# Audio-WestlakeU/FN-SSL

Measured on AMD Instinct MI355X. Metric: TF-frames/sec DP-IPD forward, 4-mic 257-bin x 300-frame, higher is better.
Workload: dtype f32; 1 GPU; BASELINE configs[1]: FN-SSL (online) DP-IPD forward, waveform->STFT->features->3x(full-band BiLSTM + narrow-band LSTM)->head; 32 utterances/GPU x 4 mics ('MM' = 6 pairs) x 257 bins x 300 frames, fp32; frame = one STFT frame of one utterance; stream_chunk_frames=0, utterances_per_gpu=32, global_batch=32, mics=4, pairs_per_utterance=6, frames=300, bins=257, parallelism=dp1 (utterance shards, no collective), chunk_pairs=0

## Files before the change

fn-ssl_amd/csrc/lstm_f32c.h:

```cpp
#pragma once

#include "lstm_static.h"

namespace fnssl_lstm {

constexpr int kF32cWaves = 16;

struct F32ClusterParams {
  unsigned* tags;
  unsigned* status;
  int clusters_per_dir;
  int groups_per_cluster;
  unsigned spin_limit;
  int stall_member;
  int rotate;
  int prio_mode;
};

template <int HH, int NV0, int NS0, int MODE, bool ABLRT = false, int DRIFT = 2, int NW_ = kF32cWaves, int GS = 1>
__global__ void __launch_bounds__(NW_ * 64) lstm_f32c_kernel(const LstmParams p, const F32ClusterParams cp) {
  constexpr int H = HH, NS = H / 16, NW = NW_;
  constexpr int NWS = NW / GS;
  static_assert((GS == 1 || GS == 4) && NW % GS == 0 && (NWS & (NWS - 1)) == 0, "gate split: whole slots, a power of two of them");
  constexpr bool SUM = (MODE & kSum) != 0, SAVE = (MODE & kSave) != 0;
  constexpr bool CAT = (MODE & kHas2) != 0;
  constexpr int QPS = 1 + NV0 + NS0 + NS;
  constexpr int XD = NW_ > 12 ? 4 : 8;
  constexpr bool STRH = H == 256 && GS == 1 && NW_ > 8;
  static_assert((CAT ? NS0 == 1 : !(NV0 && NS0)) && (NV0 == 0 || NV0 % XD == 0) && (H == 128 || H == 256),
                "blocks of src0, or its remainder alone, or blocks of src0 + the remainder quad of src2");
  static_assert(H == 128 || NW_ <= 8 || STRH, "H = 256 with the row of h_{t-1} held: at most two waves per SIMD (register budget)");
  static_assert(!STRH || (NV0 >= XD && (NV0 + NS) % XD == 0), "streamed row: the ring depth divides the block count");
  static_assert(GS == 1 || (!SAVE && !ABLRT), "gate split: inference kernels only");
  extern __shared__ __attribute__((aligned(16))) char smem[];
  const int ABL = ABLRT ? p.ablate : 0;

  const int b = blockIdx.x;
  const int m = (b >> 3) % NS;
  const int cl = ((b >> 3) / NS) * 8 + (b & 7);
  if (cl >= cp.clusters_per_dir * p.ndir) return;
  const int dir = cl / cp.clusters_per_dir;
  const int ck = cl - dir * cp.clusters_per_dir;
  const int g0 = ck * cp.groups_per_cluster;
  const int g1 = g0 + cp.groups_per_cluster < p.ntasks ? g0 + cp.groups_per_cluster : p.ntasks;
  if (__hip_atomic_load(cp.status, __ATOMIC_RELAXED, __HIP_MEMORY_SCOPE_AGENT) != 0) return;
  if (cl == 0 && m == cp.stall_member) return;

  const int lane = threadIdx.x & 63;
  const int n = lane & 15, g = lane >> 4;
  const int w = __builtin_amdgcn_readfirstlane((int)(threadIdx.x >> 6));
  const int ws = GS == 1 ? w : (w >> 2);
  const int gate = GS == 1 ? 0 : (w & 3);
  const bool rev = dir == 1;
  const unsigned vlane = lane * 16;

  {
    const v4f* src = reinterpret_cast<const v4f*>(reinterpret_cast<const char*>(p.wpack[dir]) + (size_t)(m * QPS) * 4096);
    v4f* dst = reinterpret_cast<v4f*>(smem);
    for (int i = threadIdx.x; i < QPS * 4 * 64; i += NW * 64) dst[i] = src[i];
  }
  char* const xch = smem + QPS * 4096;
  unsigned* const xcnt = reinterpret_cast<unsigned*>(xch + NWS * 2 * 4 * 1024);
  if (GS > 1 && threadIdx.x < NWS) xcnt[threadIdx.x] = 0;
  __syncthreads();
  const char* const lds_rd = smem + lane * 16;
  auto rec = [&](int q, int j) { return *reinterpret_cast<const v4f*>(lds_rd + (q * 4 + j) * 1024); };
  auto rec1 = [&](int q, int j) { return *reinterpret_cast<const float*>(lds_rd + (q * 4 + j) * 1024 + 4 * gate); };

  const unsigned st0 = (unsigned)(p.src0.st * 4), sto = (unsigned)(p.out_st * 4), stk = SUM ? (unsigned)(p.skip.st * 4) : 0u;
  const unsigned st2 = CAT ? (unsigned)(p.src2.st * 4) : 0u;
  const unsigned cy = (unsigned)p.carry;
  unsigned* const tag_cl = cp.tags + (size_t)cl * cp.groups_per_cluster * NS;
  const v4f zero4 = v4f{0.f, 0.f, 0.f, 0.f};

  unsigned pub_val = 0;
  unsigned* pub_tag = nullptr;
  auto pub_flush = [&]() {
    if (pub_tag) {
      asm volatile("s_waitcnt vmcnt(0)" ::: "memory");
      if (lane == 0) __hip_atomic_store(pub_tag, pub_val, __ATOMIC_RELAXED, __HIP_MEMORY_SCOPE_AGENT);
      pub_tag = nullptr;
    }
  };

  struct Grp {
    unsigned vo0, voo, vok, voo2, vo2 = 0;
    bool valid;
    int task, step;
  };
  auto locate = [&](int task, int qo0, int qi0, Grp& gr, rsrc_t& rx0, rsrc_t& ro, rsrc_t& rsk, rsrc_t& ro2, rsrc_t& rx2) {
    const int q0 = task * 16;
    gr.valid = q0 + n < p.nseq;
    const int d = q0 + n < p.nseq ? n : p.nseq - 1 - q0;
    const bool crossed = qi0 + d >= p.q_inner;
    auto one = [&](const float* base, long long so, long long si, int extra, unsigned& voff) {
      const long long delta = (long long)d * si + (crossed ? so - (long long)p.q_inner * si : 0ll);
      voff = (unsigned)(delta * 4) + (unsigned)(extra * 4);
      return make_rsrc(base + ((long long)qo0 * so + (long long)qi0 * si));
    };
    rx0 = one(p.src0.p, p.src0.so, p.src0.si, (NS0 && !CAT) ? g : 4 * g, gr.vo0);
    if constexpr (CAT) rx2 = one(p.src2.p, p.src2.so, p.src2.si, g, gr.vo2);
    ro = one(p.out, p.out_so, p.out_si, dir * H + 4 * g, gr.voo);
    gr.vok = gr.voo2 = 0;
    rsk = SUM ? one(p.skip.p, p.skip.so, p.skip.si, dir * H + 4 * g, gr.vok) : rx0;
    ro2 = SUM ? one(p.out_sum, p.out_so, p.out_si, dir * H + 4 * g, gr.voo2) : ro;
  };
  auto tt_of = [&](int step) { return (unsigned)(rev ? p.nsteps - 1 - step : step); };
  auto rc_of = [&](int task) {
    return make_rsrc(cell_record<NS>(p.cscratch, p.ntasks, dir, task));
  };

  if (g0 + ws >= g1) return;
  unsigned long long clk0 = 0, rt0 = 0;
  if (ABLRT && (ABL & 512)) {
    clk0 = __builtin_amdgcn_s_memtime();
    rt0 = __builtin_amdgcn_s_memrealtime();
  }
  bool dead = false;
  auto bounded_wait = [&](auto ready, auto reload, int sleep, unsigned code) {
    for (unsigned spins = 0; !ready(); ++spins) {
      if (GS > 1) __builtin_amdgcn_s_sleep(1); else if (sleep == 8) __builtin_amdgcn_s_sleep(8); else __builtin_amdgcn_s_sleep(16);
      reload();
      const bool out = spins > cp.spin_limit;
      if (out || (spins & 63) == 63) {
        if (out) {
          if (lane == 0) __hip_atomic_store(cp.status, code | (unsigned)(cl & 0xffff), __ATOMIC_RELAXED, __HIP_MEMORY_SCOPE_AGENT);
          return false;
        }
        if (__hip_atomic_load(cp.status, __ATOMIC_RELAXED, __HIP_MEMORY_SCOPE_AGENT) != 0) return false;
      }
    }
    return true;
  };
  const int NGR = g1 - g0;
  const bool rot = cp.rotate && NGR >= 2 * NWS;
  const int FULL = rot ? (NGR / NWS) * NWS : NGR, LEFT = NGR - FULL;
  const bool single = GS == 1 && g0 + ws + NWS >= g1;
  Grp cur, nxt;
  rsrc_t rx0, ro, rsk, ro2, rx2, nrx0, nro, nrsk, nro2, nrx2;
  v4f xr[XD];
  float xs0 = 0.f;
  v4f cprev = zero4, skipv = zero4;
  unsigned tagv = 0, tagd = 0;
  auto request = [&](const Grp& gr, rsrc_t qx0, rsrc_t qsk, bool with_c, bool with_x = true) {
    const unsigned tt = tt_of(gr.step);
    if (!(ABL & 8)) {
      if constexpr (NV0 > 0) if (with_x) static_for<XD>([&](auto v) { xr[v.value] = bld4(qx0, gr.vo0, tt * st0 + 64 * v.value); });
      if constexpr (NS0 > 0 && !CAT) xs0 = bld1(qx0, gr.vo0, tt * st0);
    }
    if (SUM && !(ABL & 64)) skipv = bld4(qsk, gr.vok, tt * stk + 64 * m);
    if (gr.step > 0 || cy) {
      if (gr.step > 0 && !(ABL & 256))
        tagv = __hip_atomic_load(tag_cl + (size_t)(gr.task - g0) * NS + (lane & (NS - 1)), __ATOMIC_RELAXED, __HIP_MEMORY_SCOPE_AGENT);
      if (GS == 1 && with_c && !(ABL & 64)) cprev = bld4_l2(rc_of(gr.task), vlane, m * 1024);
    }
    if (DRIFT > 0 && !(ABL & 256) && gr.task - DRIFT * NWS >= g0)
      tagd = __hip_atomic_load(tag_cl + (size_t)(gr.task - DRIFT * NWS - g0) * NS + (lane & (NS - 1)), __ATOMIC_RELAXED, __HIP_MEMORY_SCOPE_AGENT);
  };
  cur.task = g0 + ws;
  cur.step = 0;
  unsigned iter = 0;
  const int qo_first = (cur.task * 16) / p.q_inner, qi_first = cur.task * 16 - qo_first * p.q_inner;
  int qo0 = qo_first, qi0 = qi_first;
  locate(cur.task, qo0, qi0, cur, rx0, ro, rsk, ro2, rx2);
  request(cur, rx0, rsk, true);
  if constexpr (CAT) xs0 = bld1(rx2, cur.vo2, tt_of(0) * st2);

  for (;;) {
    const int step = cur.step, task = cur.task;
    const unsigned tt = tt_of(step);
    const unsigned o0 = tt * st0, oo = (tt + cy) * sto;
    const unsigned op = (rev ? tt + 1 : tt - 1 + cy) * sto;
    const rsrc_t rc = rc_of(task);
    unsigned* const tag_g = tag_cl + (size_t)(task - g0) * NS;
    if (single && (step > 0 || cy) && !(ABL & 64)) cprev = bld4_l2(rc, vlane, m * 1024);
    const bool late_c = GS > 1 || task >= g0 + FULL;
    v4f cprev_cur = (step > 0 || cy) ? cprev : zero4;
    const v4f skip_cur = skipv;

    v4f hold[STRH ? 1 : NS];
    auto fetch_h = [&]() {
      if (DRIFT > 0 && !(ABL & 4) && !dead && task - DRIFT * NWS >= g0) {
        unsigned* const tag_d = tag_cl + (size_t)(task - DRIFT * NWS - g0) * NS;
        dead = !bounded_wait([&]() { return __builtin_amdgcn_ballot_w64(tagd < (unsigned)step + 1) == 0; },
                             [&]() { tagd = __hip_atomic_load(tag_d + (lane & (NS - 1)), __ATOMIC_RELAXED, __HIP_MEMORY_SCOPE_AGENT); }, 8, 0x40000u);
      }
      if ((step > 0 || cy) && !(ABL & 16)) {
        if (step > 0 && !(ABL & 4) && !dead)
          dead = !bounded_wait([&]() { return __builtin_amdgcn_ballot_w64(tagv < (unsigned)step) == 0; },
                               [&]() { tagv = __hip_atomic_load(tag_g + (lane & (NS - 1)), __ATOMIC_RELAXED, __HIP_MEMORY_SCOPE_AGENT); }, 16, 0x30000u);
        if (late_c && !(ABL & 64)) cprev_cur = bld4_l2(rc, vlane, m * 1024);
        if constexpr (!STRH) {
#pragma unroll
          for (int s = 0; s < NS; ++s) hold[s] = bld4_l2(ro, cur.voo, op + 64 * s);
        }
      } else if constexpr (!STRH) {
#pragma unroll
        for (int s = 0; s < NS; ++s) hold[s] = (ABL & 16) ? cprev : zero4;
      }
    };
    const bool hrow = step > 0 || cy;
    auto hblock = [&](int j) { return hrow ? bld4_l2(ro, cur.voo, op + 64 * j) : zero4; };

    if (cp.prio_mode == 2) __builtin_amdgcn_s_setprio(2);
    v4f acc[4];
    v4f ra[4];
    v4f acc1 = zero4;
    float rb[4] = {0.f, 0.f, 0.f, 0.f};
    if constexpr (GS == 1) {
      acc[0] = rec(0, 0);
      acc[1] = rec(0, 1);
      acc[2] = rec(0, 2);
      acc[3] = rec(0, 3);
      static_for<4>([&](auto j) { ra[j.value] = rec(1, j.value); });
    } else {
      acc1 = rec(0, gate);
      static_for<4>([&](auto j) { rb[j.value] = rec1(1, j.value); });
    }
    auto quad = [&](auto qc, float b0, float b1, float b2, float b3) {
      constexpr int Q = decltype(qc)::value;
      if constexpr (GS > 1) {
        acc1 = __builtin_amdgcn_mfma_f32_16x16x4f32(rb[0], b0, acc1, 0, 0, 0);
        if constexpr (Q + 1 < QPS) rb[0] = rec1(Q + 1, 0);
        acc1 = __builtin_amdgcn_mfma_f32_16x16x4f32(rb[1], b1, acc1, 0, 0, 0);
        if constexpr (Q + 1 < QPS) rb[1] = rec1(Q + 1, 1);
        acc1 = __builtin_amdgcn_mfma_f32_16x16x4f32(rb[2], b2, acc1, 0, 0, 0);
        if constexpr (Q + 1 < QPS) rb[2] = rec1(Q + 1, 2);
        acc1 = __builtin_amdgcn_mfma_f32_16x16x4f32(rb[3], b3, acc1, 0, 0, 0);
        if constexpr (Q + 1 < QPS) rb[3] = rec1(Q + 1, 3);
        return;
      }
      MFMA4(acc, ra[0], b0);
      __builtin_amdgcn_sched_barrier(0);
      if constexpr (Q + 1 < QPS) if (!(ABL & 128)) ra[0] = rec(Q + 1, 0);
      __builtin_amdgcn_sched_barrier(0);
      MFMA4(acc, ra[1], b1);
      __builtin_amdgcn_sched_barrier(0);
      if constexpr (Q + 1 < QPS) if (!(ABL & 128)) ra[1] = rec(Q + 1, 1);
      __builtin_amdgcn_sched_barrier(0);
      MFMA4(acc, ra[2], b2);
      __builtin_amdgcn_sched_barrier(0);
      if constexpr (Q + 1 < QPS) if (!(ABL & 128)) ra[2] = rec(Q + 1, 2);
      __builtin_amdgcn_sched_barrier(0);
      MFMA4(acc, ra[3], b3);
      __builtin_amdgcn_sched_barrier(0);
      if constexpr (Q + 1 < QPS) if (!(ABL & 128)) ra[3] = rec(Q + 1, 3);
      __builtin_amdgcn_sched_barrier(0);
    };
    auto quad1 = [&](auto qc, float b0) {
      constexpr int Q = decltype(qc)::value;
      if constexpr (GS > 1) {
        acc1 = __builtin_amdgcn_mfma_f32_16x16x4f32(rb[0], b0, acc1, 0, 0, 0);
        if constexpr (Q + 1 < QPS) static_for<4>([&](auto j) { rb[j.value] = rec1(Q + 1, j.value); });
        return;
      }
      MFMA4(acc, ra[0], b0);
      if constexpr (Q + 1 < QPS) static_for<4>([&](auto j) { ra[j.value] = rec(Q + 1, j.value); });
    };
    if constexpr (NV0 > 0) {
      static_for<NV0>([&](auto v) {
        constexpr int V = decltype(v)::value;
        if constexpr (STRH) {
          if constexpr (V == NV0 / 2) pub_flush();
          if constexpr (V == NV0 - XD) fetch_h();
        } else if constexpr (V == NV0 / 2) {
          pub_flush();
          fetch_h();
        }
        const v4f xb = xr[V % XD];
        quad(ic<1 + V>{}, xb.x, xb.y, xb.z, xb.w);
        if constexpr (V + XD < NV0) {
          if (!(ABL & 8)) xr[V % XD] = bld4(rx0, cur.vo0, o0 + 64 * (V + XD));
        } else if constexpr (STRH) {
          xr[V % XD] = hblock(V + XD - NV0);
        }
      });
      if constexpr (NS0 > 0) quad1(ic<1 + NV0>{}, xs0);
    } else {
      pub_flush();
      fetch_h();
      quad1(ic<1>{}, xs0);
    }
    bool seq_next = false;
    if (task < g0 + FULL && task + NWS < g0 + FULL) {
      nxt.task = task + NWS;
      nxt.step = step;
      seq_next = true;
    } else {
      const int j = (ws - step) & (NWS - 1);
      if (task < g0 + FULL && j < LEFT) {
        nxt.task = g0 + FULL + j;
        nxt.step = step;
      } else {
        nxt.task = g0 + ws;
        nxt.step = step + 1;
      }
    }
    const bool more = nxt.step < p.nsteps;
    if (more) {
      if (ABL & 1) {
        nxt.vo0 = cur.vo0; nxt.voo = cur.voo; nxt.vok = cur.vok; nxt.voo2 = cur.voo2; nxt.valid = cur.valid;
        nrx0 = rx0; nro = ro; nrsk = rsk; nro2 = ro2;
        if constexpr (CAT) {
          nxt.vo2 = cur.vo2;
          nrx2 = rx2;
        }
      } else {
        if (seq_next) {
          qi0 += 16 * NWS;
          while (qi0 >= p.q_inner) {
            qi0 -= p.q_inner;
            ++qo0;
          }
        } else if (nxt.step == step) {
          qo0 = (nxt.task * 16) / p.q_inner;
          qi0 = nxt.task * 16 - qo0 * p.q_inner;
        } else {
          qo0 = qo_first;
          qi0 = qi_first;
        }
        locate(nxt.task, qo0, qi0, nxt, nrx0, nro, nrsk, nro2, nrx2);
      }
      request(nxt, nrx0, nrsk, !single && nxt.task < g0 + FULL, !STRH);
      if constexpr (CAT) xs0 = bld1(nrx2, nxt.vo2, tt_of(nxt.step) * st2);
    }
    static_for<NS>([&](auto sp) {
      constexpr int SP = decltype(sp)::value;
      if constexpr (STRH) {
        constexpr int B = NV0 + SP, B2 = B + XD;
        const v4f hb = xr[B % XD];
        quad(ic<1 + NV0 + NS0 + SP>{}, hb.x, hb.y, hb.z, hb.w);
        if constexpr (B2 < NV0 + NS) {
          xr[B % XD] = hblock(B2 - NV0);
        } else {
          if (more) xr[B % XD] = bld4(nrx0, nxt.vo0, tt_of(nxt.step) * st0 + 64 * (B2 - NV0 - NS));
        }
      } else {
        quad(ic<1 + NV0 + NS0 + SP>{}, hold[SP].x, hold[SP].y, hold[SP].z, hold[SP].w);
      }
    });

    if (cp.prio_mode == 2) __builtin_amdgcn_s_setprio(0);
    if (dead) break;
    v4f cn, hn;
    if (ABL & 2) {
      cn = acc[1] + cprev_cur + acc[0];
      hn = acc[3] + acc[2];
    } else {
      v4f ig, fg, gg, og;
      if constexpr (GS == 1) {
        ig = sigmoid4(acc[0]);
        fg = sigmoid4(acc[1]);
        gg = tanh4(acc[2]);
        og = sigmoid4(acc[3]);
      } else {
        const v4f act = gate == 2 ? tanh4(acc1) : sigmoid4(acc1);
        v4f* const xb = reinterpret_cast<v4f*>(xch + (size_t)((ws * 2 + (int)(iter & 1u)) * 4) * 1024);
        xb[gate * 64 + lane] = act;
        asm volatile("s_waitcnt lgkmcnt(0)" ::: "memory");
        if (lane == 0) __hip_atomic_fetch_add(xcnt + ws, 1u, __ATOMIC_RELAXED, __HIP_MEMORY_SCOPE_WORKGROUP);
        const unsigned want = 4u * (iter + 1u);
        for (unsigned spins = 0;; ++spins) {
          if (__hip_atomic_load(xcnt + ws, __ATOMIC_RELAXED, __HIP_MEMORY_SCOPE_WORKGROUP) >= want) break;
          if (dead || ((spins & 63u) == 63u && __hip_atomic_load(cp.status, __ATOMIC_RELAXED, __HIP_MEMORY_SCOPE_AGENT) != 0u) ||
              spins > cp.spin_limit) {
            dead = true;
            break;
          }
          __builtin_amdgcn_s_sleep(1);
        }
        asm volatile("" ::: "memory");
        ig = xb[lane];
        fg = xb[64 + lane];
        gg = xb[128 + lane];
        og = xb[192 + lane];
        ++iter;
      }
      cn = cell4(fg, cprev_cur, ig, gg);
      hn = mul_rn4(og, tanh4(cn));
      if constexpr (SAVE) {
        const rsrc_t rres = make_rsrc(reinterpret_cast<const char*>(p.reserve) +
                                      ((size_t)dir * p.ntasks + task) * p.nsteps * (size_t)(NS * kReserveRecs * 1024));
        const unsigned rb = (tt * NS + m) * (kReserveRecs * 1024);
        bst4(ig, rres, vlane, rb);
        bst4(fg, rres, vlane, rb + 1024);
        bst4(gg, rres, vlane, rb + 2048);
        bst4(og, rres, vlane, rb + 3072);
        bst4(cn, rres, vlane, rb + 4096);
      }
    }
    asm("" : "+v"(hn.x), "+v"(hn.y), "+v"(hn.z), "+v"(hn.w));
    if (ABL & 32) asm volatile("" ::"v"(cn), "v"(hn));
    const bool storer = GS == 1 || gate == 0;
    if (storer && !(ABL & 32)) bst4(cn, rc, vlane, m * 1024);
    if (storer && cur.valid && !(ABL & 32)) {
      __builtin_amdgcn_raw_buffer_store_b128(__builtin_bit_cast(v4u, hn), ro, cur.voo, oo + 64 * m, 16);
      if (SUM) bst4(add_rn4(hn, skip_cur), ro2, cur.voo2, oo + 64 * m);
    }
    pub_val = __builtin_amdgcn_readfirstlane((unsigned)step + 1);
    pub_tag = ((ABL & 256) || !storer) ? nullptr : tag_g + m;
    if (GS > 1 || single) pub_flush();
    if (!more || dead) break;
    cur = nxt;
    rx0 = nrx0;
    ro = nro;
    rsk = nrsk;
    ro2 = nro2;
    if constexpr (CAT) rx2 = nrx2;
  }
  pub_flush();
  asm volatile("s_waitcnt vmcnt(0)" ::: "memory");
  if (ABLRT && (ABL & 512) && (w == 0 || w == 15) && lane == 0) {
    const unsigned long long c1 = __builtin_amdgcn_s_memtime(), r1 = __builtin_amdgcn_s_memrealtime();
    printf("f32c blk %d wave %d start %llu end %llu cycles %llu MHz %.1f\n", b, w, rt0, r1, c1 - clk0,
           (double)(c1 - clk0) / (double)(r1 - rt0) * 100.0);
  }
}

template <int HH, int NV0, int NS0, int MODE, bool ABLRT = false, int DRIFT = 2, int NW_ = kF32cWaves, int GS = 1>
int launch_f32c_k(const LstmParams& p, const F32ClusterParams& cp, const LaunchCtx& lc) {
  constexpr int NS = HH / 16;
  constexpr int QPS = 1 + NV0 + NS0 + NS;
  const size_t lds = (size_t)QPS * 4096 + (GS > 1 ? (size_t)(NW_ / GS) * 8192 + 64 : 0);
  static_assert(QPS * 4096 + (GS > 1 ? (NW_ / GS) * 8192 + 64 : 0) <= 160 * 1024, "LDS");
  const int ncl = cp.clusters_per_dir * p.ndir;
  const int nwg = 8 * NS * ((ncl + 7) / 8);
  return enqueue(lc, Kernel{lstm_f32c_kernel<HH, NV0, NS0, MODE, ABLRT, DRIFT, NW_, GS>, NW_ * 64, lds, "lstm_f32c_kernel", true}, nwg, p, cp);
}

}
```

fn-ssl_amd/csrc/lstm_f32c.hip:

```cpp
#include <cstdlib>

#include "lstm_f32c.h"
#include "tuning.h"

namespace fnssl_lstm {

constexpr int kF32cWavesH256 = 16;
constexpr int kF32cWavesH256Split = 8;

static bool f32c_uniform(const LstmParams& p, int mode) {
  auto even = [&](long long so, long long si) { return si >= 0 && so == (long long)p.q_inner * si; };
  return even(p.src0.so, p.src0.si) && even(p.out_so, p.out_si) && (!(mode & kSum) || even(p.skip.so, p.skip.si)) &&
         (!(mode & kHas2) || even(p.src2.so, p.src2.si));
}

bool f32c_handles(const LstmParams& p, int H, int mode) {
  if (fnssl::tune(FNSSL_TUNE_NO_F32_CLUSTER)) return false;
  if ((H != 128 && H != 256) || p.ablate) return false;
  if (H == 128) {
    if (p.c2 != 0 || p.carry) return false;
    if (p.reserve && mode != 0) return false;
    if (!(p.c0 == 256 && (mode == kSum || mode == 0)) && !(p.c0 == 4 && mode == 0 && !fnssl::tune(FNSSL_TUNE_NO_F32C_B1))) return false;
  } else {
    if (p.ndir != 1 || p.c0 != 256 || fnssl::tune(FNSSL_TUNE_NO_F32_SMALL)) return false;
    const bool plain = p.c2 == 0 && (mode == 0 || mode == kSum), cat = p.c2 == 4 && (mode == kHas2 || mode == (kHas2 | kSum));
    if (!plain && !cat) return false;
    if (p.reserve && ((mode & kSum) || p.carry)) return false;
  }
  auto grows = [&](long long so, long long si) { return si >= 0 && so >= (long long)(p.q_inner - 1) * si; };
  if (!f32c_uniform(p, mode) &&
      (p.q_inner < 16 || !grows(p.src0.so, p.src0.si) || !grows(p.out_so, p.out_si) ||
       ((mode & kSum) && !grows(p.skip.so, p.skip.si)) || ((mode & kHas2) && !grows(p.src2.so, p.src2.si))))
    return false;
  const int ncu = cluster_cus();
  if (ncu < (H / 16) * p.ndir) return false;
  const long long groups = (long long)p.ntasks * p.ndir;
  if (const int mg = fnssl::tune(FNSSL_TUNE_F32C_MIN_GROUPS, 1, 1 << 30)) {
    if (groups < mg) return false;
  }
  if (p.reserve) {
    if (fnssl::tune(FNSSL_TUNE_TRAIN_NO_F32_CLUSTER)) return false;
    return true;
  }
  if (H == 256) {
    const long long full = 12LL * ncu, rounds = (groups + full - 1) / full;
    return groups < full || groups * 100 < rounds * full * 97;
  }
  return !fnssl::tune(FNSSL_TUNE_NO_F32_SMALL) || groups >= 12LL * ncu;
}

template <int NW_, int GS>
static int launch_f32c_h256(const LstmParams& p, const F32ClusterParams& cp, int mode, const LaunchCtx& lc) {
  if (mode == (kHas2 | kSum)) return launch_f32c_k<256, 16, 1, kHas2 | kSum, false, 2, NW_, GS>(p, cp, lc);
  if (mode == kHas2) return launch_f32c_k<256, 16, 1, kHas2, false, 2, NW_, GS>(p, cp, lc);
  if (mode == kSum) return launch_f32c_k<256, 16, 0, kSum, false, 2, NW_, GS>(p, cp, lc);
  return launch_f32c_k<256, 16, 0, 0, false, 2, NW_, GS>(p, cp, lc);
}

int forward_f32c(LstmParams p, int H, int mode, size_t cluster_bytes, const LaunchCtx& lc) {
  if (f32c_uniform(p, mode)) p.q_inner = p.nseq;
  const int ncu = cluster_cus();
  const int members = H / 16;
  F32ClusterParams cp;
  cp.clusters_per_dir = (ncu / members) / p.ndir;
  cp.groups_per_cluster = (p.ntasks + cp.clusters_per_dir - 1) / cp.clusters_per_dir;
  cp.status = reinterpret_cast<unsigned*>(p.cluster_ws);
  cp.tags = reinterpret_cast<unsigned*>(p.cluster_ws + 256);
  cp.spin_limit = cluster_spin_limit();
  cp.stall_member = cluster_test_stall();
  cp.rotate = !fnssl::tune(FNSSL_TUNE_F32C_NO_ROTATE);
  cp.prio_mode = fnssl::tune(FNSSL_TUNE_F32C_PRIO, 9, 9) ? 0 : 2;
  const size_t tag_bytes = (size_t)p.ndir * cp.clusters_per_dir * cp.groups_per_cluster * members * sizeof(unsigned);
  FNSSL_REQUIRE(256 + tag_bytes <= cluster_bytes, "lstm_forward: the cluster kernel's tags exceed the workspace's cluster area");
  if (!lc.dry) FNSSL_HIP(hipMemsetAsync(p.cluster_ws, 0, 256 + tag_bytes, lc.st));
  const int gs_knob = fnssl::tune(FNSSL_TUNE_F32C_GATE_SPLIT, 1, 4);
  const bool gsplit = gs_knob ? gs_knob == 4 : cp.groups_per_cluster <= 1;
  if (H == 256) {
    constexpr int W = kF32cWavesH256;
    if (p.reserve)
      return p.c2 == 4 ? launch_f32c_k<256, 16, 1, kHas2 | kSave, false, 2, W>(p, cp, lc) : launch_f32c_k<256, 16, 0, kSave, false, 2, W>(p, cp, lc);
    if (gsplit) return launch_f32c_h256<kF32cWavesH256Split, 4>(p, cp, mode, lc);
    if (cp.groups_per_cluster <= kF32cWavesH256Split) return launch_f32c_h256<kF32cWavesH256Split, 1>(p, cp, mode, lc);
    return launch_f32c_h256<W, 1>(p, cp, mode, lc);
  }
  if (gsplit && !p.reserve) {
    if (p.c0 == 4) return launch_f32c_k<128, 0, 1, 0, false, 2, kF32cWaves, 4>(p, cp, lc);
    if (mode == kSum) return launch_f32c_k<128, 16, 0, kSum, false, 2, kF32cWaves, 4>(p, cp, lc);
    return launch_f32c_k<128, 16, 0, 0, false, 2, kF32cWaves, 4>(p, cp, lc);
  }
#ifdef FNSSL_BUILD_ABLATE
  if (const int abl = env_int("FNSSL_F32C_ABL", 1, 1023)) {
    p.ablate = abl;
    if (mode == kSum) return launch_f32c_k<128, 16, 0, kSum, true>(p, cp, lc);
    if (p.c0 == 4) return launch_f32c_k<128, 0, 1, 0, true>(p, cp, lc);
  }
  p.ablate = 0;
#endif
  if (p.reserve) return p.c0 == 4 ? launch_f32c_k<128, 0, 1, kSave>(p, cp, lc) : launch_f32c_k<128, 16, 0, kSave>(p, cp, lc);
  if (p.c0 == 4) return launch_f32c_k<128, 0, 1, 0>(p, cp, lc);
  if (mode == kSum) return launch_f32c_k<128, 16, 0, kSum>(p, cp, lc);
  return launch_f32c_k<128, 16, 0, 0>(p, cp, lc);
}

}
```

Measured before the change: 17810 frames/s.

## Use cluster-wide buffer descriptors with incremental offsets in the f32 cluster LSTM kernel

Result: no change. 17840 frames/s (median of 3 runs) (+0.2%).

```diff
diff --git a/fn-ssl_amd/csrc/lstm_f32c.h b/fn-ssl_amd/csrc/lstm_f32c.h
--- a/fn-ssl_amd/csrc/lstm_f32c.h
+++ b/fn-ssl_amd/csrc/lstm_f32c.h
@@ -15,7 +15,12 @@
   int stall_member;
   int rotate;
   int prio_mode;
+  int geom;
 };
+
+constexpr int kGeoSkipAsSrc0 = 1;
+constexpr int kGeoEvenOut = 2;
+constexpr int kGeoEvenSrc0 = 4;
 
 template <int HH, int NV0, int NS0, int MODE, bool ABLRT = false, int DRIFT = 2, int NW_ = kF32cWaves, int GS = 1>
 __global__ void __launch_bounds__(NW_ * 64) lstm_f32c_kernel(const LstmParams p, const F32ClusterParams cp) {
@@ -63,9 +68,19 @@
   unsigned* const xcnt = reinterpret_cast<unsigned*>(xch + NWS * 2 * 4 * 1024);
   if (GS > 1 && threadIdx.x < NWS) xcnt[threadIdx.x] = 0;
   __syncthreads();
-  const char* const lds_rd = smem + lane * 16;
-  auto rec = [&](int q, int j) { return *reinterpret_cast<const v4f*>(lds_rd + (q * 4 + j) * 1024); };
-  auto rec1 = [&](int q, int j) { return *reinterpret_cast<const float*>(lds_rd + (q * 4 + j) * 1024 + 4 * gate); };
+  typedef const char __attribute__((address_space(3))) * lds_cptr;
+  lds_cptr lds_rd[3];
+  lds_rd[0] = (lds_cptr)smem + (GS > 1 ? lane * 16 + 4 * gate : lane * 16);
+  lds_rd[1] = lds_rd[0] + 65536;
+  lds_rd[2] = lds_rd[0] + 2 * 65536;
+  if constexpr (QPS * 4096 > 65536) asm("" : "+v"(lds_rd[1]));
+  if constexpr (QPS * 4096 > 2 * 65536) asm("" : "+v"(lds_rd[2]));
+  auto rec_at = [&](int q, int j) {
+    const unsigned off = (unsigned)(q * 4 + j) * 1024;
+    return lds_rd[off >> 16] + (off & 65535u);
+  };
+  auto rec = [&](int q, int j) { return *reinterpret_cast<const v4f __attribute__((address_space(3)))*>(rec_at(q, j) - (GS > 1 ? 4 * gate : 0)); };
+  auto rec1 = [&](int q, int j) { return *reinterpret_cast<const float __attribute__((address_space(3)))*>(rec_at(q, j)); };
 
   const unsigned st0 = (unsigned)(p.src0.st * 4), sto = (unsigned)(p.out_st * 4), stk = SUM ? (unsigned)(p.skip.st * 4) : 0u;
   const unsigned st2 = CAT ? (unsigned)(p.src2.st * 4) : 0u;
@@ -73,44 +88,83 @@
   unsigned* const tag_cl = cp.tags + (size_t)cl * cp.groups_per_cluster * NS;
   const v4f zero4 = v4f{0.f, 0.f, 0.f, 0.f};
 
-  unsigned pub_val = 0;
-  unsigned* pub_tag = nullptr;
+  constexpr unsigned kNoTag = ~0u;
+  unsigned pub_val = 0, pub_tag = kNoTag;
   auto pub_flush = [&]() {
-    if (pub_tag) {
+    if (pub_tag != kNoTag) {
       asm volatile("s_waitcnt vmcnt(0)" ::: "memory");
-      if (lane == 0) __hip_atomic_store(pub_tag, pub_val, __ATOMIC_RELAXED, __HIP_MEMORY_SCOPE_AGENT);
-      pub_tag = nullptr;
-    }
-  };
-
+      if (lane == 0) __hip_atomic_store(tag_cl + pub_tag, pub_val, __ATOMIC_RELAXED, __HIP_MEMORY_SCOPE_AGENT);
+      pub_tag = kNoTag;
+    }
+  };
+
+  if (g0 + ws >= g1) return;
+  static_assert(!(SUM && NS0 && !CAT), "skip rides on src0's 16-byte lane offsets");
+  const bool skip_own = SUM && !(cp.geom & kGeoSkipAsSrc0);
+  const int seq_c = g0 * 16, seq_l = (g1 * 16 < p.nseq ? g1 * 16 : p.nseq) - 1;
+  const int qo_c = seq_c / p.q_inner, qi_c = seq_c - qo_c * p.q_inner;
+  const int qo_l = seq_l / p.q_inner, qi_l = seq_l - qo_l * p.q_inner;
+  auto slice = [&](const float* base, long long so, long long si, long long st, int rows, int lead, int width) {
+    const long long first = (long long)qo_c * so + (long long)qi_c * si + lead;
+    const long long bytes = ((long long)qo_l * so + (long long)qi_l * si + lead - first + (long long)(rows - 1) * st + width) * 4;
+    return __builtin_amdgcn_make_buffer_rsrc(const_cast<float*>(base + first), 0, (unsigned)bytes, 0x00020000);
+  };
+  const rsrc_t dx0 = slice(p.src0.p, p.src0.so, p.src0.si, p.src0.st, p.nsteps, 0, NV0 ? 16 * NV0 : 4);
+  const rsrc_t dout = slice(p.out, p.out_so, p.out_si, p.out_st, p.nsteps + (int)cy, 0, p.ndir * H);
+  const rsrc_t dsum = SUM ? slice(p.out_sum, p.out_so, p.out_si, p.out_st, p.nsteps + (int)cy, 0, p.ndir * H) : dout;
+  const rsrc_t dsk = SUM ? slice(p.skip.p, p.skip.so, p.skip.si, p.skip.st, p.nsteps, dir * H + 16 * m, 16) : dx0;
+  const rsrc_t dx2 = CAT ? slice(p.src2.p, p.src2.so, p.src2.si, p.src2.st, p.nsteps, 0, 4) : dx0;
+  const rsrc_t dcell = __builtin_amdgcn_make_buffer_rsrc(const_cast<char*>(cell_record<NS>(p.cscratch, p.ntasks, dir, g0)) + m * 1024, 0,
+                                                         (unsigned)(g1 - g0 - 1) * (NS * 1024) + 1024u, 0x00020000);
+  auto cell_off = [&](int task) { return (unsigned)(task - g0) * (NS * 1024); };
+  struct Geo {
+    unsigned si, wrap, lane;
+  };
+  auto geo = [&](long long so, long long si, int extra) {
+    const unsigned si4 = (unsigned)(si * 4);
+    return Geo{si4, (unsigned)(so * 4) - (unsigned)p.q_inner * si4, (unsigned)n * si4 + (unsigned)(extra * 4)};
+  };
+  const Geo gx = geo(p.src0.so, p.src0.si, (NS0 && !CAT) ? g : 4 * g);
+  const Geo go = geo(p.out_so, p.out_si, dir * H + 4 * g);
+  const Geo gk = SUM ? geo(p.skip.so, p.skip.si, 4 * g) : gx;
+  const Geo g2 = CAT ? geo(p.src2.so, p.src2.si, g) : gx;
   struct Grp {
-    unsigned vo0, voo, vok, voo2, vo2 = 0;
-    bool valid;
+    unsigned ux, uo;
+    unsigned vx, vo;
     int task, step;
   };
-  auto locate = [&](int task, int qo0, int qi0, Grp& gr, rsrc_t& rx0, rsrc_t& ro, rsrc_t& rsk, rsrc_t& ro2, rsrc_t& rx2) {
-    const int q0 = task * 16;
-    gr.valid = q0 + n < p.nseq;
-    const int d = q0 + n < p.nseq ? n : p.nseq - 1 - q0;
-    const bool crossed = qi0 + d >= p.q_inner;
-    auto one = [&](const float* base, long long so, long long si, int extra, unsigned& voff) {
-      const long long delta = (long long)d * si + (crossed ? so - (long long)p.q_inner * si : 0ll);
-      voff = (unsigned)(delta * 4) + (unsigned)(extra * 4);
-      return make_rsrc(base + ((long long)qo0 * so + (long long)qi0 * si));
-    };
-    rx0 = one(p.src0.p, p.src0.so, p.src0.si, (NS0 && !CAT) ? g : 4 * g, gr.vo0);
-    if constexpr (CAT) rx2 = one(p.src2.p, p.src2.so, p.src2.si, g, gr.vo2);
-    ro = one(p.out, p.out_so, p.out_si, dir * H + 4 * g, gr.voo);
-    gr.vok = gr.voo2 = 0;
-    rsk = SUM ? one(p.skip.p, p.skip.so, p.skip.si, dir * H + 4 * g, gr.vok) : rx0;
-    ro2 = SUM ? one(p.out_sum, p.out_so, p.out_si, dir * H + 4 * g, gr.voo2) : ro;
+  struct Pos {
+    int qi;
+    unsigned ux, uo, uk, u2;
+  };
+  auto advance = [&](Pos& ps, int groups) {
+    ps.qi += 16 * groups;
+    ps.ux += 16 * groups * gx.si;
+    ps.uo += 16 * groups * go.si;
+    if (skip_own) ps.uk += 16 * groups * gk.si;
+    if constexpr (CAT) ps.u2 += 16 * groups * g2.si;
+    while (ps.qi >= p.q_inner) {
+      ps.qi -= p.q_inner;
+      ps.ux += gx.wrap;
+      ps.uo += go.wrap;
+      if (skip_own) ps.uk += gk.wrap;
+      if constexpr (CAT) ps.u2 += g2.wrap;
+    }
+  };
+  auto lane_off = [&](const Geo& ge, bool even, int task, int qi) {
+    const int live = p.nseq - task * 16;
+    if (live >= 16) return (!even && n >= p.q_inner - qi) ? ge.lane + ge.wrap : ge.lane;
+    const int d = n < live ? n : live - 1;
+    return ge.lane + (unsigned)(d - n) * ge.si + (d >= p.q_inner - qi ? ge.wrap : 0u);
+  };
+  auto locate = [&](int task, const Pos& ps, Grp& gr) {
+    gr.ux = ps.ux;
+    gr.uo = ps.uo;
+    gr.vx = lane_off(gx, (cp.geom & kGeoEvenSrc0) != 0, task, ps.qi);
+    gr.vo = lane_off(go, (cp.geom & kGeoEvenOut) != 0, task, ps.qi);
   };
   auto tt_of = [&](int step) { return (unsigned)(rev ? p.nsteps - 1 - step : step); };
-  auto rc_of = [&](int task) {
-    return make_rsrc(cell_record<NS>(p.cscratch, p.ntasks, dir, task));
-  };
-
-  if (g0 + ws >= g1) return;
+
   unsigned long long clk0 = 0, rt0 = 0;
   if (ABLRT && (ABL & 512)) {
     clk0 = __builtin_amdgcn_s_memtime();
@@ -137,22 +191,25 @@
   const int FULL = rot ? (NGR / NWS) * NWS : NGR, LEFT = NGR - FULL;
   const bool single = GS == 1 && g0 + ws + NWS >= g1;
   Grp cur, nxt;
-  rsrc_t rx0, ro, rsk, ro2, rx2, nrx0, nro, nrsk, nro2, nrx2;
   v4f xr[XD];
   float xs0 = 0.f;
   v4f cprev = zero4, skipv = zero4;
   unsigned tagv = 0, tagd = 0;
-  auto request = [&](const Grp& gr, rsrc_t qx0, rsrc_t qsk, bool with_c, bool with_x = true) {
+  auto request = [&](const Grp& gr, const Pos& ps, bool with_c, bool with_x = true) {
     const unsigned tt = tt_of(gr.step);
     if (!(ABL & 8)) {
-      if constexpr (NV0 > 0) if (with_x) static_for<XD>([&](auto v) { xr[v.value] = bld4(qx0, gr.vo0, tt * st0 + 64 * v.value); });
-      if constexpr (NS0 > 0 && !CAT) xs0 = bld1(qx0, gr.vo0, tt * st0);
-    }
-    if (SUM && !(ABL & 64)) skipv = bld4(qsk, gr.vok, tt * stk + 64 * m);
+      if constexpr (NV0 > 0) if (with_x) static_for<XD>([&](auto v) { xr[v.value] = bld4(dx0, gr.vx, gr.ux + tt * st0 + 64 * v.value); });
+      if constexpr (NS0 > 0 && !CAT) xs0 = bld1(dx0, gr.vx, gr.ux + tt * st0);
+    }
+    if (SUM && !(ABL & 64)) {
+      if (skip_own) skipv = bld4(dsk, lane_off(gk, false, gr.task, ps.qi), ps.uk + tt * stk);
+      else skipv = bld4(dsk, gr.vx, gr.ux + tt * stk);
+    }
+    if constexpr (CAT) xs0 = bld1(dx2, lane_off(g2, false, gr.task, ps.qi), ps.u2 + tt * st2);
     if (gr.step > 0 || cy) {
       if (gr.step > 0 && !(ABL & 256))
         tagv = __hip_atomic_load(tag_cl + (size_t)(gr.task - g0) * NS + (lane & (NS - 1)), __ATOMIC_RELAXED, __HIP_MEMORY_SCOPE_AGENT);
-      if (GS == 1 && with_c && !(ABL & 64)) cprev = bld4_l2(rc_of(gr.task), vlane, m * 1024);
+      if (GS == 1 && with_c && !(ABL & 64)) cprev = bld4_l2(dcell, vlane, cell_off(gr.task));
     }
     if (DRIFT > 0 && !(ABL & 256) && gr.task - DRIFT * NWS >= g0)
       tagd = __hip_atomic_load(tag_cl + (size_t)(gr.task - DRIFT * NWS - g0) * NS + (lane & (NS - 1)), __ATOMIC_RELAXED, __HIP_MEMORY_SCOPE_AGENT);
@@ -160,20 +217,20 @@
   cur.task = g0 + ws;
   cur.step = 0;
   unsigned iter = 0;
-  const int qo_first = (cur.task * 16) / p.q_inner, qi_first = cur.task * 16 - qo_first * p.q_inner;
-  int qo0 = qo_first, qi0 = qi_first;
-  locate(cur.task, qo0, qi0, cur, rx0, ro, rsk, ro2, rx2);
-  request(cur, rx0, rsk, true);
-  if constexpr (CAT) xs0 = bld1(rx2, cur.vo2, tt_of(0) * st2);
+  const Pos cluster_base{qi_c, 0u, 0u, 0u, 0u};
+  Pos pos = cluster_base;
+  advance(pos, ws);
+  locate(cur.task, pos, cur);
+  request(cur, pos, true);
 
   for (;;) {
     const int step = cur.step, task = cur.task;
     const unsigned tt = tt_of(step);
-    const unsigned o0 = tt * st0, oo = (tt + cy) * sto;
-    const unsigned op = (rev ? tt + 1 : tt - 1 + cy) * sto;
-    const rsrc_t rc = rc_of(task);
+    const unsigned o0 = cur.ux + tt * st0, oo = cur.uo + (tt + cy) * sto;
+    const unsigned op = cur.uo + (rev ? tt + 1 : tt - 1 + cy) * sto;
+    const unsigned oc = cell_off(task);
     unsigned* const tag_g = tag_cl + (size_t)(task - g0) * NS;
-    if (single && (step > 0 || cy) && !(ABL & 64)) cprev = bld4_l2(rc, vlane, m * 1024);
+    if (single && (step > 0 || cy) && !(ABL & 64)) cprev = bld4_l2(dcell, vlane, oc);
     const bool late_c = GS > 1 || task >= g0 + FULL;
     v4f cprev_cur = (step > 0 || cy) ? cprev : zero4;
     const v4f skip_cur = skipv;
@@ -189,10 +246,10 @@
         if (step > 0 && !(ABL & 4) && !dead)
           dead = !bounded_wait([&]() { return __builtin_amdgcn_ballot_w64(tagv < (unsigned)step) == 0; },
                                [&]() { tagv = __hip_atomic_load(tag_g + (lane & (NS - 1)), __ATOMIC_RELAXED, __HIP_MEMORY_SCOPE_AGENT); }, 16, 0x30000u);
-        if (late_c && !(ABL & 64)) cprev_cur = bld4_l2(rc, vlane, m * 1024);
+        if (late_c && !(ABL & 64)) cprev_cur = bld4_l2(dcell, vlane, oc);
         if constexpr (!STRH) {
 #pragma unroll
-          for (int s = 0; s < NS; ++s) hold[s] = bld4_l2(ro, cur.voo, op + 64 * s);
+          for (int s = 0; s < NS; ++s) hold[s] = bld4_l2(dout, cur.vo, op + 64 * s);
         }
       } else if constexpr (!STRH) {
 #pragma unroll
@@ -200,7 +257,7 @@
       }
     };
     const bool hrow = step > 0 || cy;
-    auto hblock = [&](int j) { return hrow ? bld4_l2(ro, cur.voo, op + 64 * j) : zero4; };
+    auto hblock = [&](int j) { return hrow ? bld4_l2(dout, cur.vo, op + 64 * j) : zero4; };
 
     if (cp.prio_mode == 2) __builtin_amdgcn_s_setprio(2);
     v4f acc[4];
@@ -270,7 +327,7 @@
         const v4f xb = xr[V % XD];
         quad(ic<1 + V>{}, xb.x, xb.y, xb.z, xb.w);
         if constexpr (V + XD < NV0) {
-          if (!(ABL & 8)) xr[V % XD] = bld4(rx0, cur.vo0, o0 + 64 * (V + XD));
+          if (!(ABL & 8)) xr[V % XD] = bld4(dx0, cur.vx, o0 + 64 * (V + XD));
         } else if constexpr (STRH) {
           xr[V % XD] = hblock(V + XD - NV0);
         }
@@ -281,11 +338,9 @@
       fetch_h();
       quad1(ic<1>{}, xs0);
     }
-    bool seq_next = false;
     if (task < g0 + FULL && task + NWS < g0 + FULL) {
       nxt.task = task + NWS;
       nxt.step = step;
-      seq_next = true;
     } else {
       const int j = (ws - step) & (NWS - 1);
       if (task < g0 + FULL && j < LEFT) {
@@ -299,30 +354,17 @@
     const bool more = nxt.step < p.nsteps;
     if (more) {
       if (ABL & 1) {
-        nxt.vo0 = cur.vo0; nxt.voo = cur.voo; nxt.vok = cur.vok; nxt.voo2 = cur.voo2; nxt.valid = cur.valid;
-        nrx0 = rx0; nro = ro; nrsk = rsk; nro2 = ro2;
-        if constexpr (CAT) {
-          nxt.vo2 = cur.vo2;
-          nrx2 = rx2;
-        }
+        nxt.ux = cur.ux; nxt.uo = cur.uo; nxt.vx = cur.vx; nxt.vo = cur.vo;
       } else {
-        if (seq_next) {
-          qi0 += 16 * NWS;
-          while (qi0 >= p.q_inner) {
-            qi0 -= p.q_inner;
-            ++qo0;
-          }
-        } else if (nxt.step == step) {
-          qo0 = (nxt.task * 16) / p.q_inner;
-          qi0 = nxt.task * 16 - qo0 * p.q_inner;
+        if (nxt.step == step) {
+          advance(pos, nxt.task - task);
         } else {
-          qo0 = qo_first;
-          qi0 = qi_first;
-        }
-        locate(nxt.task, qo0, qi0, nxt, nrx0, nro, nrsk, nro2, nrx2);
-      }
-      request(nxt, nrx0, nrsk, !single && nxt.task < g0 + FULL, !STRH);
-      if constexpr (CAT) xs0 = bld1(nrx2, nxt.vo2, tt_of(nxt.step) * st2);
+          pos = cluster_base;
+          advance(pos, ws);
+        }
+        locate(nxt.task, pos, nxt);
+      }
+      request(nxt, pos, !single && nxt.task < g0 + FULL, !STRH);
     }
     static_for<NS>([&](auto sp) {
       constexpr int SP = decltype(sp)::value;
@@ -333,7 +375,7 @@
         if constexpr (B2 < NV0 + NS) {
           xr[B % XD] = hblock(B2 - NV0);
         } else {
-          if (more) xr[B % XD] = bld4(nrx0, nxt.vo0, tt_of(nxt.step) * st0 + 64 * (B2 - NV0 - NS));
+          if (more) xr[B % XD] = bld4(dx0, nxt.vx, nxt.ux + tt_of(nxt.step) * st0 + 64 * (B2 - NV0 - NS));
         }
       } else {
         quad(ic<1 + NV0 + NS0 + SP>{}, hold[SP].x, hold[SP].y, hold[SP].z, hold[SP].w);
@@ -392,21 +434,16 @@
     asm("" : "+v"(hn.x), "+v"(hn.y), "+v"(hn.z), "+v"(hn.w));
     if (ABL & 32) asm volatile("" ::"v"(cn), "v"(hn));
     const bool storer = GS == 1 || gate == 0;
-    if (storer && !(ABL & 32)) bst4(cn, rc, vlane, m * 1024);
-    if (storer && cur.valid && !(ABL & 32)) {
-      __builtin_amdgcn_raw_buffer_store_b128(__builtin_bit_cast(v4u, hn), ro, cur.voo, oo + 64 * m, 16);
-      if (SUM) bst4(add_rn4(hn, skip_cur), ro2, cur.voo2, oo + 64 * m);
+    if (storer && !(ABL & 32)) bst4(cn, dcell, vlane, oc);
+    if (storer && !(ABL & 32) && (task * 16 + 16 <= p.nseq || task * 16 + n < p.nseq)) {
+      __builtin_amdgcn_raw_buffer_store_b128(__builtin_bit_cast(v4u, hn), dout, cur.vo, oo + 64 * m, 16);
+      if (SUM) bst4(add_rn4(hn, skip_cur), dsum, cur.vo, oo + 64 * m);
     }
     pub_val = __builtin_amdgcn_readfirstlane((unsigned)step + 1);
-    pub_tag = ((ABL & 256) || !storer) ? nullptr : tag_g + m;
+    pub_tag = ((ABL & 256) || !storer) ? kNoTag : (unsigned)((task - g0) * NS + m);
     if (GS > 1 || single) pub_flush();
     if (!more || dead) break;
     cur = nxt;
-    rx0 = nrx0;
-    ro = nro;
-    rsk = nrsk;
-    ro2 = nro2;
-    if constexpr (CAT) rx2 = nrx2;
   }
   pub_flush();
   asm volatile("s_waitcnt vmcnt(0)" ::: "memory");
diff --git a/fn-ssl_amd/csrc/lstm_f32c.hip b/fn-ssl_amd/csrc/lstm_f32c.hip
--- a/fn-ssl_amd/csrc/lstm_f32c.hip
+++ b/fn-ssl_amd/csrc/lstm_f32c.hip
@@ -1,3 +1,4 @@
+#include <algorithm>
 #include <cstdlib>
 
 #include "lstm_f32c.h"
@@ -12,6 +13,31 @@
   auto even = [&](long long so, long long si) { return si >= 0 && so == (long long)p.q_inner * si; };
   return even(p.src0.so, p.src0.si) && even(p.out_so, p.out_si) && (!(mode & kSum) || even(p.skip.so, p.skip.si)) &&
          (!(mode & kHas2) || even(p.src2.so, p.src2.si));
+}
+
+static void f32c_partition(const LstmParams& p, int H, int& clusters_per_dir, int& groups_per_cluster) {
+  clusters_per_dir = (cluster_cus() / (H / 16)) / p.ndir;
+  groups_per_cluster = (p.ntasks + clusters_per_dir - 1) / clusters_per_dir;
+}
+
+static bool f32c_spans_fit(const LstmParams& p, int H, int mode) {
+  int cpd, gpc;
+  f32c_partition(p, H, cpd, gpc);
+  const long long q_inner = f32c_uniform(p, mode) ? p.nseq : p.q_inner;
+  auto fits = [&](long long so, long long si, long long st, long long rows, long long width) {
+    for (int c = 0; c < cpd; ++c) {
+      const long long s0 = (long long)c * gpc * 16, s1 = std::min<long long>(s0 + (long long)gpc * 16, p.nseq) - 1;
+      if (s1 < s0) break;
+      const long double span = (long double)(s1 / q_inner - s0 / q_inner) * so + (long double)(s1 % q_inner - s0 % q_inner) * si +
+                               (long double)rows * st + width;
+      if (span * 4.0L > 4294967295.0L) return false;
+    }
+    return true;
+  };
+  return fits(p.src0.so, p.src0.si, p.src0.st, p.nsteps, p.c0) &&
+         fits(p.out_so, p.out_si, p.out_st, p.nsteps + p.carry, (long long)p.ndir * H) &&
+         (!(mode & kSum) || fits(p.skip.so, p.skip.si, p.skip.st, p.nsteps, (long long)p.ndir * H)) &&
+         (!(mode & kHas2) || fits(p.src2.so, p.src2.si, p.src2.st, p.nsteps, p.c2));
 }
 
 bool f32c_handles(const LstmParams& p, int H, int mode) {
@@ -34,6 +60,7 @@
     return false;
   const int ncu = cluster_cus();
   if (ncu < (H / 16) * p.ndir) return false;
+  if (!f32c_spans_fit(p, H, mode)) return false;
   const long long groups = (long long)p.ntasks * p.ndir;
   if (const int mg = fnssl::tune(FNSSL_TUNE_F32C_MIN_GROUPS, 1, 1 << 30)) {
     if (groups < mg) return false;
@@ -58,12 +85,14 @@
 }
 
 int forward_f32c(LstmParams p, int H, int mode, size_t cluster_bytes, const LaunchCtx& lc) {
-  if (f32c_uniform(p, mode)) p.q_inner = p.nseq;
-  const int ncu = cluster_cus();
+  const bool uniform = f32c_uniform(p, mode);
+  if (uniform) p.q_inner = p.nseq;
   const int members = H / 16;
   F32ClusterParams cp;
-  cp.clusters_per_dir = (ncu / members) / p.ndir;
-  cp.groups_per_cluster = (p.ntasks + cp.clusters_per_dir - 1) / cp.clusters_per_dir;
+  f32c_partition(p, H, cp.clusters_per_dir, cp.groups_per_cluster);
+  auto even = [&](long long so, long long si) { return uniform || so == (long long)p.q_inner * si; };
+  cp.geom = (((mode & kSum) && p.skip.so == p.src0.so && p.skip.si == p.src0.si) ? kGeoSkipAsSrc0 : 0) |
+            (even(p.out_so, p.out_si) ? kGeoEvenOut : 0) | (even(p.src0.so, p.src0.si) ? kGeoEvenSrc0 : 0);
   cp.status = reinterpret_cast<unsigned*>(p.cluster_ws);
   cp.tags = reinterpret_cast<unsigned*>(p.cluster_ws + 256);
   cp.spin_limit = cluster_spin_limit();
```
